# dpmerrell/PathMatFac.jl

Measured on AMD Instinct MI355X. Metric: fit_iters_per_sec, higher is better.
Workload: dtype f32; 1 GPU; fit! epoch on synthetic 200000x50000 matrix (D stored as f32), K=64, Gaussian loss, group-reg X (32 groups) + featureset-ARD Y, adam; rows sharded over 1 GPU(s); full_model=False, M=200000, N=50000, K=64, rows_per_gpu=200000, optimizer=adam, parallelism=single GPU, rccl_ranks=0, collectives_issued=0, column_chunks=1

## Files before the change

pathmatfac.jl_amd/csrc/pmf_common.h:

```cpp
#ifndef PMF_COMMON_H
#define PMF_COMMON_H
#include <hip/hip_runtime.h>

#include <cstdint>
#include <type_traits>
#include <unordered_map>

#include "../../include/pmf_hip.h"

int pmf_fail(const char *fmt, ...);
#define HIPCHK(x)                                                                                    \
  do {                                                                                               \
    hipError_t e_ = (x);                                                                             \
    if (e_ != hipSuccess) return pmf_fail("%s failed: %s (%s:%d)", #x, hipGetErrorString(e_), __FILE__, __LINE__); \
  } while (0)
#define PMFCHK(x)          \
  do {                     \
    int r_ = (x);          \
    if (r_ < 0) return r_; \
  } while (0)

typedef std::unordered_map<const void *, size_t> PmfDynLds;
int pmf_ensure_dyn_lds(PmfDynLds *cache, const void *kern, size_t lds);

// ... 29 lines not shown
  float *gY;
  float *gy_slabs;
  int64_t slab_stride;
  int64_t n_rp;
  int64_t n_tiles;
  const int64_t *wg_begin;
  int32_t tps;
  int32_t n_ct;
  const float4 *colp;
  const int32_t *bor;
  const float2 *btab;
  const float2 *btd;
  const uint8_t *pm, *row_slot, *colview;
  int32_t nbs_shift;
  int32_t n_bv;
  double *loss_partial;
  int64_t M, N;
  int32_t n_cseg;
  int32_t want_gx, want_gy;
  unsigned long long *stamps;
  int32_t dbg;
  const ViewDesc *views;
  const char *Xsb, *Ysb;
  int32_t ct0;
  float *gx_part;
  const int32_t *piece_base;
  int64_t gx_slot_stride;
  const float *sb_scale_x, *sb_scale_y;
};

__device__ __forceinline__ int pmf_rowmap(int r, int h) { return (r & 3) + 8 * (r >> 2) + 4 * h; }
__device__ __forceinline__ bool pmf_finite(float y) { return fabsf(y) <= 3.402823466e38f; }

__device__ __forceinline__ void pmf_noise(int kind, float z, float y, float w, float &l, float &g) {
  if (kind == PMF_NOISE_NORMAL) {
    const float d = z - y;
    g = w * d;
    l = 0.5f * g * d;
  } else if (kind == PMF_NOISE_BERNOULLI) {
    const float e = __expf(-fabsf(z));
    const float sp = fmaxf(z, 0.f) + __logf(1.f + e);
    const float r = __frcp_rn(1.f + e);
    const float sg = z >= 0.f ? r : e * r;
    l = w * (sp - y * z);
    g = w * (sg - y);
  } else {
// ... 249 lines not shown
```

pathmatfac.jl_amd/csrc/pmf_ctx.h:

```cpp
#ifndef PMF_CTX_H
#define PMF_CTX_H
#include <hip/hip_runtime.h>

#include <algorithm>
#include <chrono>
#include <cmath>
#include <cstdarg>
#include <cstdio>
#include <cstdlib>
#include <cstring>
#include <string>
#include <unordered_map>
#include <vector>

#include "pmf_common.h"

struct ParamBuf {
  float *p = nullptr, *g = nullptr, *acc = nullptr, *mom = nullptr;
  float *wq = nullptr, *cq = nullptr;
  float *wl1 = nullptr;
  int64_t n = 0;
  float bp1 = 0.f, bp2 = 0.f;
};

// ... 104 lines not shown
  bool has_ard = false;
  bool ard_is_fsard = false;
  int opt_kind = PMF_OPT_ADAGRAD;
  float lr = 1.f, eps = 1e-8f, b1 = 0.9f, b2 = 0.999f;
  bool state_init = false;
  double *loss_partial = nullptr;
  std::vector<uint8_t> h_kind;
  std::vector<WorkSplit> splits;
  int n_chunks_req = 0;
  float *gx_part = nullptr;
  size_t gx_part_cap = 0;
  int32_t *gx_off = nullptr, *gx_idx = nullptr;
  int64_t gx_serial = -1;
  int64_t split_serial = 0;
  Comm comm;
  int last_chunks = 1;
  hipEvent_t ev_host = nullptr;
  int64_t kind_version = 0;
  float *gy_slabs = nullptr;
  size_t gy_slabs_cap = 0;
  int precision = PMF_PREC_F32;
  char *xsb = nullptr, *ysb = nullptr;
  size_t xsb_cap = 0, ysb_cap = 0;
  float *sb8_scale = nullptr;
  uint32_t *sb8_max = nullptr;
  int64_t sb_launches = 0;
  int64_t loss_cap = 0;
  int64_t n_macro = 0;
  double *reg_partial = nullptr;
  double *d_loss = nullptr;
  double *h_loss = nullptr;
  std::vector<std::pair<hipEvent_t, hipEvent_t>> ev_pool;
  size_t ev_used = 0;
  double kernel_ms_sum = 0.0;
  int64_t kernel_launches = 0;
  NetReg *net[2] = {nullptr, nullptr};
  int reg_counts[4] = {0, 0, 0, 0};
  void *scratch = nullptr;
  size_t scratch_bytes = 0;
  PmfDynLds dyn_lds;
};

#define REG_SLOTS 1024
#define PMF_MAX_CHUNKS 16

struct FusedFamily;
// ... 61 lines not shown
```

pathmatfac.jl_amd/csrc/pmf_fused.hip.inc:

```

template <int KB, int NW, int RBW = 1>
struct FusedCfg {
  static constexpr int Kp = 32 * KB;
  static constexpr int KpS = Kp + 4;
  static constexpr int SLAB = 32 * Kp;
  static constexpr int YT = PMF_BN * KpS;
  static constexpr int XP = 32 * KpS;
  static constexpr int TT = (RBW - 1) * 1024;
  static constexpr int FIXED = NW * SLAB + NW * RBW * XP + NW * TT + 8 * PMF_BN + 4;
  static constexpr int LDS_BUDGET = 160 * 1024;
  static constexpr int NYB = (2 * YT + FIXED) * 4 + 8 * NW <= LDS_BUDGET ? 2 : 1;
  static constexpr size_t lds_bytes = (sizeof(float) * (NYB * YT + FIXED) + sizeof(double) * NW + 15) / 16 * 16;
  static constexpr size_t lds_batch_extra = PMF_BN * 16 * sizeof(float2) + PMF_PM_BYTES + NW * RBW * 16 * 32;
};

#ifndef PMF_NW4_WAVES
#define PMF_NW4_WAVES 1
#endif
template <int KB, int NW, int RBW, int BMODE, bool MIXED, int GM, bool DB, bool XW = false>
__global__ __launch_bounds__(64 * NW, (NW == 8 ? 2 : PMF_NW4_WAVES)) void pmf_fused_kernel(const FusedArgs a) {
  using Cfg = FusedCfg<KB, NW, RBW>;
  constexpr bool FULL = GM != 3;
  constexpr bool BATCH = BMODE != 0;
  constexpr bool bt_lds = BMODE == 1;
// ... 36 lines not shown
  const int dbg = FULL ? 0 : a.dbg;
  float *Sw = Sl + w * SLAB;
  float *Xw[RBW], *T[RBW];
#pragma unroll
  for (int rb = 0; rb < RBW; ++rb) {
    Xw[rb] = Xs + (w * RBW + rb) * Cfg::XP;
    T[rb] = rb == 0 ? Sw + (KB - 1) * 1024 : Tt + (w * (RBW - 1) + rb - 1) * 1024;
  }
  const int xw_j = 16 * (w & 1) + (lane & 15), xw_k = 16 * (w >> 1) + 4 * (lane >> 4);
  const int xw_e = xw_j * Kp + xw_k;
  const int xw_x = 4 * (lane >> 4) * KpS + 16 * (w >> 1) + (lane & 15);
  int xw_g[4];
  typedef const __attribute__((address_space(3))) float *lds_cptr;
  unsigned xw_xa[4];
#pragma unroll
  for (int u = 0; u < 4; ++u) {
    const int i = 4 * (lane >> 4) + u;
    xw_g[u] = i * 32 + 4 * ((xw_j >> 2) ^ (i & 7)) + (xw_j & 3);
    xw_xa[u] = (unsigned)(uintptr_t)(lds_cptr)(Xs + xw_x + u * KpS);
    if (XW) asm volatile("" : "+v"(xw_xa[u]));
  }

  constexpr bool HOIST = KB == 2 && NW == 8 && RBW == 1 && GM != 3 && (XW || GM != 0 || BMODE == 0);
  unsigned ho_y[2][YV], ho_s[2][YV], ho_c[2], ho_g[2][RV4];
  if (HOIST) {
#pragma unroll
    for (int z = 0; z < 2; ++z) {
      const int ncol = z == 0 || N % BN == 0 ? BN : (int)(N % BN);
#pragma unroll
      for (int q = 0; q < YV; ++q) {
        int e4 = tid + NT * q;
        if (e4 > BN * Kp / 4 - 1) e4 = BN * Kp / 4 - 1;
        int jl = (e4 * 4) / Kp;
        if (jl >= ncol) { jl = ncol - 1; e4 = jl * (Kp / 4); }
        ho_y[z][q] = 16u * e4;
        ho_s[z][q] = 16u * jl;
        asm volatile("" : "+v"(ho_y[z][q]), "+v"(ho_s[z][q]));
      }
      ho_c[z] = 16u * (tid < ncol ? tid : ncol - 1);
      asm volatile("" : "+v"(ho_c[z]));
#pragma unroll
      for (int q = 0; q < RV4; ++q) {
        int e = xw_e;
        if (!XW) {
          const int f = tid + NT * q, ff = f < BN * Kp / 4 ? f : 0;
          e = ((ff % (BN * 8)) / 8) * Kp + 32 * (ff / (BN * 8)) + 4 * (ff % 8);
        }
        ho_g[z][q] = 4u * (e < ncol * Kp ? e : e % Kp);
        asm volatile("" : "+v"(ho_g[z][q]));
      }
    }
  }
  auto ho_at = [](const void *base, unsigned off) { return reinterpret_cast<const char *>(base) + off; };
#ifdef PMF_STAMPS
  unsigned long long st_acc[16] = {0, 0, 0, 0, 0, 0, 0, 0, 0, 0, 0, 0, 0, 0, 0, 0};
  unsigned long long st_prev = __builtin_amdgcn_s_memtime();
  const unsigned long long st_t0 = st_prev, st_r0 = __builtin_amdgcn_s_memrealtime();
#endif
  const int wg = pmf_xcd_wg(blockIdx.x, gridDim.x);
  const int64_t w_begin = a.wg_begin[wg];
  const int64_t w_end = a.wg_begin[wg + 1];
// ... 24 lines not shown
      irow_c[rb] = row_ok[rb] ? irow : (M - 1);
    }

    constexpr int XV = (32 * Kp / 4) / 64;
    float4 xv0[RBW][XV];
#pragma unroll
    for (int rb = 0; rb < RBW; ++rb) {
#pragma unroll
      for (int q = 0; q < XV; ++q) {
        const int e4 = lane + 64 * q;
        const int il = (e4 * 4) / Kp;
        const int64_t ir = row0[rb] + il < M ? row0[rb] + il : M - 1;
        xv0[rb][q] = *reinterpret_cast<const float4 *>(a.X + ir * Kp + (e4 * 4) % Kp);
      }
    }
    f32x16 gx[RBW][KB];
#pragma unroll
    for (int rb = 0; rb < RBW; ++rb)
#pragma unroll
      for (int kb = 0; kb < KB; ++kb)
#pragma unroll
        for (int r = 0; r < 16; ++r) gx[rb][kb][r] = 0.f;

    auto stage_load_y = [&](int64_t jt, int q, float4 (&yv)[YV], float (&sgv)[YV]) {
      const float *yb = a.Y + jt * Kp;
      const float4 *cb = a.colp + jt;
      const int64_t rem = N - jt;
      if (HOIST) {
        const bool rag = rem < BN;
        yv[q] = *reinterpret_cast<const float4 *>(ho_at(yb, rag ? ho_y[1][q] : ho_y[0][q]));
        sgv[q] = *reinterpret_cast<const float *>(ho_at(cb, rag ? ho_s[1][q] : ho_s[0][q]));
        return;
      }
      const int ncol = rem > BN ? BN : (int)rem;
      int e4 = tid + NT * q;
      if (e4 > BN * Kp / 4 - 1) e4 = BN * Kp / 4 - 1;
      int jl = (e4 * 4) / Kp;
      if (jl >= ncol) { jl = ncol - 1; e4 = jl * (Kp / 4); }
      yv[q] = *reinterpret_cast<const float4 *>(yb + e4 * 4);
      sgv[q] = cb[jl].x;
    };
    auto stage_load_c = [&](int64_t jt, float4 &cv) {
      const float4 *cb = a.colp + jt;
      const int64_t rem = N - jt;
      if (HOIST) {
        cv = *reinterpret_cast<const float4 *>(ho_at(cb, rem < BN ? ho_c[1] : ho_c[0]));
        return;
      }
      const int ncol = rem > BN ? BN : (int)rem;
      cv = cb[tid < ncol ? tid : ncol - 1];
    };
    auto stage_load = [&](int64_t jt, float4 (&yv)[YV], float (&sgv)[YV], float4 &cv) {
#pragma unroll
      for (int q = 0; q < YV; ++q) stage_load_y(jt, q, yv, sgv);
      stage_load_c(jt, cv);
    };
    auto stage_store = [&](int ybuf, int cbuf, int64_t jt, const float4 (&yv)[YV], const float (&sgv)[YV], const float4 &cv) {
      float *Yn = Ys + ybuf * Cfg::YT;
      const int64_t rem = N - jt;
      const int ncol = rem > BN ? BN : (int)rem;
#pragma unroll
      for (int q = 0; q < YV; ++q) {
        const int e4 = tid + NT * q;
        if (e4 < BN * Kp / 4) {
          const int jl = (e4 * 4) / Kp, kf = (e4 * 4) % Kp;
          const float sg = jl < ncol ? sgv[q] : 0.f;
          *reinterpret_cast<float4 *>(Yn + jl * KpS + kf) = make_float4(yv[q].x * sg, yv[q].y * sg, yv[q].z * sg, yv[q].w * sg);
        }
      }
      asm volatile("" ::"v"(cv.x), "v"(cv.y), "v"(cv.z), "v"(cv.w));
      if (tid < BN) {
        const bool livec = tid < ncol;
        Csg[cbuf * BN + tid] = livec ? cv.x : 0.f;
        Cmu[cbuf * BN + tid] = livec ? cv.y : 0.f;
        Cw[cbuf * BN + tid] = livec ? cv.z : 0.f;
        Cmt[cbuf * BN + tid] = livec ? __float_as_int(cv.w) : 3;
        if (MIXED) {
          const int kd = __float_as_int(cv.w) & 3;
          const unsigned m0 = (unsigned)__ballot(!livec || kd == 0), m1 = (unsigned)__ballot(!livec || kd == 1),
                         m2 = (unsigned)__ballot(!livec || kd == 2);
          if (tid == 0) Ck[cbuf] = m0 == 0xffffffffu ? 0 : (m1 == 0xffffffffu ? 1 : (m2 == 0xffffffffu ? 2 : 3));
        }
        if (bt_lds) {
          const int vw = (__float_as_int(cv.w) >> 2) - 1;
          const int vw0 = __builtin_amdgcn_readfirstlane(vw);
          const unsigned mv = (unsigned)__ballot(!livec || vw == vw0);
          if (tid == 0) Ck[2 + cbuf] = mv == 0xffffffffu ? vw0 : -2;
        }
      }
    };
// ... 100 lines not shown
          float4 v = racc[q];
          const float sgj = Csg[(cbuf ^ 1) * BN + eo[q] / Kp];
          v.x *= sgj; v.y *= sgj; v.z *= sgj; v.w *= sgj;
          if (!slab_first) { v.x += gold[q].x; v.y += gold[q].y; v.z += gold[q].z; v.w += gold[q].w; }
          if (in[q] && eo[q] < nel) pmf_store_stream(reinterpret_cast<float4 *>(sb + eo[q]), v);
        }
      }
    };

    bool rows_in[RBW];
    int rb_u[RBW];
    uint32_t tflag[RBW];
#pragma unroll
    for (int rb = 0; rb < RBW; ++rb) {
      const int rb_raw = __builtin_amdgcn_readfirstlane((int)(row0[rb] >> 5));
      rows_in[rb] = rb_raw < a.nRB;
      rb_u[rb] = rows_in[rb] ? rb_raw : (int)a.nRB - 1;
      tflag[rb] = a.tflags[(col_begin >> 5) * a.nRB + rb_u[rb]];
#pragma unroll
      for (int q = 0; q < DCH; ++q) dcur[rb].load(a.D, (col_begin >> 5) * a.nRB + rb_u[rb], lane, q);
    }
    {
      float4 yv[YV], cv;
      float sgv[YV];
      stage_load(col_begin, yv, sgv, cv);
#pragma unroll
      for (int rb = 0; rb < RBW; ++rb)
#pragma unroll
        for (int q = 0; q < XV; ++q) {
          const int e4 = lane + 64 * q;
          const int il = (e4 * 4) / Kp, kf = (e4 * 4) % Kp;
          *reinterpret_cast<float4 *>(Xw[rb] + il * KpS + kf) = row0[rb] + il < M ? xv0[rb][q] : make_float4(0.f, 0.f, 0.f, 0.f);
        }
      stage_store(0, 0, col_begin, yv, sgv, cv);
      if (bt_lds) {
#pragma unroll
        for (int q = 0; q < NBT; ++q) {
          const int e = bt_e(q);
          bt_store(e, pmf_bt_entry(a, a.pm + rp * a.n_bv * 16, col_begin, e, pmf_bt_view(a, col_begin, e)), bt_mu(col_begin, e));
        }
        if (tid < a.n_bv * 16) Pm[tid] = a.pm[rp * a.n_bv * 16 + tid];
        if (h == 0)
#pragma unroll
          for (int rb = 0; rb < RBW; ++rb)
            for (int v = 0; v < a.n_bv; ++v) Bw0[rb * 512 + v * 32 + l31] = a.row_slot[(int64_t)v * M + irow_c[rb]];
      }
    }
    __syncthreads();

    f32x16 acc[RBW];
    forward_reduce(acc, 0, 0, false, 0);

    for (int t = 0; t < ntiles; ++t) {
      const int par = t & 1;
      const int cur = NYB == 2 ? par : 0, nxt = NYB == 2 ? (par ^ 1) : 0;
      const int64_t j0 = col_begin + (int64_t)t * BN;
      const float *Yc = Ys + cur * Cfg::YT;
      const bool have_next = (t + 1 < ntiles);
      const int cb0 = par * BN + 4 * h;
      float4 ynext[YV], cnext;
      float2 btn[NBT];
      float btm[NBT];
      int btv[NBT];
      float sgnext[YV];
      PMF_STAMP(0);
      const float xw_sg = XW ? Csg[par * BN + xw_j] : 0.f;

      float lsum = 0.f;
      const int tkind = MIXED ? __builtin_amdgcn_readfirstlane(Ck[par]) : 0;
      const int tview = bt_lds ? __builtin_amdgcn_readfirstlane(Ck[2 + par]) : -1;
      float lnorm = 0.f;
      auto epi_reg = [&](int rb, int r, float dl, float th, float wj, int kmode, bool fast) __attribute__((always_inline)) {
        if (dbg & 4) return;
        float z = acc[rb][r];
        if (BATCH) z = fmaf(z, dl, th);
        float y = dcur[rb].get(r);
        if (kmode == PMF_NOISE_NORMAL) {
          if (!fast) y = (pmf_finite(y) && row_ok[rb]) ? y : z;
          const float d = z - y, g = wj * d;
          lnorm = fmaf(g, d, lnorm);
          acc[rb][r] = BATCH ? g * dl : g;
        } else {
          const bool ok = pmf_finite(y) && row_ok[rb];
          float l, g;
          if (kmode == 3) pmf_noise(Cmt[cb0 + (r & 3) + 8 * (r >> 2)] & 3, z, y, wj, l, g);
          else pmf_noise(kmode, z, y, wj, l, g);
          lsum += ok ? l : 0.f;
          acc[rb][r] = ok ? (BATCH ? g * dl : g) : 0.f;
        }
// ... 27 lines not shown
                  tv[u] += dt.y;
                }
              }
            }
          }
          dl4 = make_float4(dv[0], dv[1], dv[2], dv[3]);
          th4 = make_float4(tv[0], tv[1], tv[2], tv[3]);
        }
      };
      const float4 *cw4 = reinterpret_cast<const float4 *>(Cw + cb0);
      auto f4get = [](const float4 &v, int u) { return u == 0 ? v.x : (u == 1 ? v.y : (u == 2 ? v.z : v.w)); };

      const int64_t jn = have_next ? j0 + BN : j0;
      constexpr int NOTH = YV + 1 + RV4 + (BATCH ? NBT : 0);
      constexpr int NVM = NOTH + (DCH + 1) * RBW;
      bool tile_fast[RBW];
#pragma unroll
      for (int rb = 0; rb < RBW; ++rb) tile_fast[rb] = rows_in[rb] && tflag[rb] != 0;
      auto vmem_op = [&](int i) {
        if (i == 0 && bt_lds) {
#pragma unroll
          for (int q = 0; q < NBT; ++q) btv[q] = pmf_bt_view(a, jn, bt_e(q));
        }
        if (i < YV) stage_load_y(jn, i, ynext, sgnext);
        else if (i == YV) stage_load_c(jn, cnext);
        else if (i < YV + 1 + RV4) { if (want_gy) slab_prefetch_one(j0, i - YV - 1); }
        else if (i < NOTH) {
          const int q = i - YV - 1 - RV4;
          if (bt_lds) { btn[q] = pmf_bt_entry(a, Pm, jn, bt_e(q), btv[q]); btm[q] = bt_mu(jn, bt_e(q)); }
        }
        else if (i < NVM) {
          const int rb = (i - NOTH) / (DCH + 1), q = (i - NOTH) % (DCH + 1);
          if (q < DCH) {
            if (FULL || !(dbg & 2)) dcur[rb].load(a.D, (jn >> 5) * a.nRB + rb_u[rb], lane, q);
          } else {
            tflag[rb] = a.tflags[(jn >> 5) * a.nRB + rb_u[rb]];
          }
        }
      };
      typedef float f32x2 __attribute__((ext_vector_type(2)));
#pragma unroll
      for (int rb = 0; rb < RBW; ++rb) {
        if (!BATCH && tile_fast[rb] && (!MIXED || tkind == 0)) {
          f32x2 ls2 = {0.f, 0.f};
          if (!(dbg & 4)) {
#pragma unroll
            for (int c4 = 0; c4 < 4; ++c4) {
// ... 92 lines not shown
            for (int kb = 0; kb < KB; ++kb)
              gy[kb] = __builtin_amdgcn_mfma_f32_32x32x2f32(av, Xw[rb][i * KpS + 32 * kb + l31], gy[kb], 0, 0, 0);
          }
        }
        if (GM == 2) {
#pragma unroll
          for (int i = 16; i < NVM; ++i) vmem_op(i);
        }
        if (!(dbg & 32)) {
#pragma unroll
          for (int kb = 0; kb < KB; ++kb)
#pragma unroll
            for (int r = 0; r < 16; ++r) Sw[kb * 1024 + pmf_rowmap(r, h) * 32 + l31] = gy[kb][r];
        } else {
          f32x16 keep = gy[0];
#pragma unroll
          for (int kb = 1; kb < KB; ++kb) keep += gy[kb];
          asm volatile("" ::"v"(keep));
        }
      }

      PMF_STAMP(4);
      if (NYB == 1) __syncthreads();
      stage_store(nxt, par ^ 1, jn, ynext, sgnext, cnext);
      PMF_STAMP(5);
      __syncthreads();
      PMF_STAMP(6);

      if (bt_lds) {
#pragma unroll
        for (int q = 0; q < NBT; ++q) bt_store(bt_e(q), btn[q], btm[q]);
      }
      slab_first = pidx == 0 || (pidx == 1 && ti0 + t < t0_first);
      if (XW) {
        typedef float f32x4 __attribute__((ext_vector_type(4)));
        constexpr int XW_RING = 8, XW_AHEAD = 6;
        const float *Gp = Sl + par * (NW * 1024);
        float xa[XW_RING], xb[XW_RING];
        auto xw_read = [&](int q) __attribute__((always_inline)) {
          const int p = q >> 3, u = (q >> 1) & 3;
#pragma unroll
          for (int hi = 0; hi < 2; ++hi) {
            xa[(q + hi) % XW_RING] = *(lds_cptr)(uintptr_t)(xw_xa[u] + 4 * (p * Cfg::XP + 16 * hi * KpS));
            xb[(q + hi) % XW_RING] = Gp[p * 1024 + xw_g[u] + 512 * hi];
          }
        };
#pragma unroll
        for (int q = 0; q < XW_AHEAD; q += 2) xw_read(q);
        f32x4 gy0 = {0.f, 0.f, 0.f, 0.f}, gy1 = {0.f, 0.f, 0.f, 0.f};
        __builtin_amdgcn_sched_barrier(0);
#pragma unroll
        for (int q = 0; q < 8 * NW; q += 2) {
          if (q + XW_AHEAD < 8 * NW) xw_read(q + XW_AHEAD);
          gy0 = __builtin_amdgcn_mfma_f32_16x16x4f32(xa[q % XW_RING], xb[q % XW_RING], gy0, 0, 0, 0);
          gy1 = __builtin_amdgcn_mfma_f32_16x16x4f32(xa[(q + 1) % XW_RING], xb[(q + 1) % XW_RING], gy1, 0, 0, 0);
          __builtin_amdgcn_sched_barrier(0);
        }
        dcur[0].touch();
        const int64_t rem = N - j0;
        const int nel = (rem > BN ? BN : (int)rem) * Kp;
        float4 v = make_float4((gy0[0] + gy1[0]) * xw_sg, (gy0[1] + gy1[1]) * xw_sg, (gy0[2] + gy1[2]) * xw_sg, (gy0[3] + gy1[3]) * xw_sg);
        if (!slab_first) { v.x += gold[0].x; v.y += gold[0].y; v.z += gold[0].z; v.w += gold[0].w; }
        if (xw_e < nel) pmf_store_stream(reinterpret_cast<float4 *>(myslab + j0 * Kp + xw_e), v);
        PMF_STAMP(4);
        forward_reduce(acc, nxt, par ^ 1, false, 0);
        PMF_STAMP(8);
        if (bt_lds) __syncthreads();
        PMF_STAMP(9);
      } else {
        if (FULL || have_next) forward_reduce(acc, nxt, par ^ 1, want_gy && !(dbg & 1), j0);
        else if (want_gy && !(dbg & 1)) { f32x16 dummy[RBW]; forward_reduce(dummy, nxt, par ^ 1, true, j0); }
        PMF_STAMP(8);
        if ((GM != 1 || bt_lds) && !(dbg & 16)) __syncthreads();
        PMF_STAMP(9);
      }
    }
    if (XW && !bt_lds) __syncthreads();

    PMF_STAMP(10);
    if (want_gx) {
      float *gp = a.gx_part + (int64_t)gx_slot * a.gx_slot_stride + (int64_t)(w * RBW) * 32 * Kp + l31;
#pragma unroll
      for (int rb = 0; rb < RBW; ++rb)
#pragma unroll
        for (int kb = 0; kb < KB; ++kb)
#pragma unroll
          for (int r = 0; r < 16; ++r) gp[(rb * 32 + pmf_rowmap(r, h)) * Kp + 32 * kb] = gx[rb][kb][r];
    }
// ... 21 lines not shown
```

pathmatfac.jl_amd/csrc/pmf_hip.hip:

```cpp
#include "pmf_ctx.h"

static thread_local std::string g_err;
int pmf_fail(const char *fmt, ...) {
  char buf[1024];
  va_list ap;
  va_start(ap, fmt);
  vsnprintf(buf, sizeof(buf), fmt, ap);
  va_end(ap);
  g_err = buf;
  return -1;
}
extern "C" const char *pmf_last_error(void) { return g_err.c_str(); }
extern "C" int pmf_version(void) { return 1; }


int ctx_bind(pmf_ctx *c) {
  if (!c) return pmf_fail("null context");
  HIPCHK(hipSetDevice(c->device));
  return 0;
}

int memset_now(void *p, int v, size_t bytes) {
  HIPCHK(hipMemset(p, v, bytes));
  HIPCHK(hipStreamSynchronize(nullptr));
// ... 16 lines not shown
  b.n = 0;
}

int pmf_ensure_dyn_lds(PmfDynLds *cache, const void *kern, size_t lds) {
  auto it = cache->find(kern);
  if (it != cache->end() && it->second >= lds) return 0;
  HIPCHK(hipFuncSetAttribute(kern, hipFuncAttributeMaxDynamicSharedMemorySize, (int)lds));
  (*cache)[kern] = lds;
  return 0;
}
int ensure_dyn_lds(pmf_ctx *c, const void *kern, size_t lds) { return pmf_ensure_dyn_lds(&c->dyn_lds, kern, lds); }

static int ensure_scratch(pmf_ctx *c, size_t bytes) {
  if (c->scratch_bytes >= bytes) return 0;
  if (c->scratch) HIPCHK(hipFree(c->scratch));
  c->scratch = nullptr;
  HIPCHK(hipMalloc(&c->scratch, bytes));
  c->scratch_bytes = bytes;
  return 0;
}

__global__ void k_fill(float *p, int64_t n, float v) {
  for (int64_t e = blockIdx.x * (int64_t)blockDim.x + threadIdx.x; e < n; e += (int64_t)gridDim.x * blockDim.x) p[e] = v;
}

__global__ void k_prepare(const float *logsigma, const float *mu, const float *colw, const int32_t *colmeta,
                          float4 *colp, int64_t N, const float *logdelta, const float *theta, float2 *btab,
                          int64_t nbt) {
  const int64_t e = blockIdx.x * (int64_t)blockDim.x + threadIdx.x;
  if (e < N) colp[e] = make_float4(expf(logsigma[e]), mu[e], colw[e], __int_as_float(colmeta[e]));
  if (e < nbt) btab[e] = make_float2(expf(logdelta[e]), theta[e]);
}

struct DenseBtabArgs {
  const int32_t *colmeta;
  const float2 *btab;
  float2 *btd;
  uint8_t *colview;
  int64_t N, Npad;
  int32_t nbs_shift;
  ViewDesc views[PMF_MAXV];
};
__global__ void k_dense_btab(const DenseBtabArgs a) {
  const int64_t e = blockIdx.x * (int64_t)blockDim.x + threadIdx.x;
  if (e >= (a.Npad << a.nbs_shift)) return;
  const int64_t j = e >> a.nbs_shift;
// ... 598 lines not shown
  HIPCHK(hipMalloc((void **)&c->d_loss, sizeof(double) * 8));
  HIPCHK(hipHostMalloc((void **)&c->h_loss, sizeof(double) * 8));
  HIPCHK(hipMalloc((void **)&c->reg_partial, sizeof(double) * 4 * REG_SLOTS));
  PMFCHK(memset_now(c->reg_partial, 0, sizeof(double) * 4 * REG_SLOTS));
  {
    const char *pe = getenv("PMF_PRECISION");
    if (pe && std::string(pe) == "bf16x3") c->precision = PMF_PREC_BF16X3;
  }
  *out = c;
  return 0;
}

extern "C" int pmf_destroy(pmf_ctx *c) {
  if (!c) return 0;
  (void)hipSetDevice(c->device);
  (void)hipStreamSynchronize(c->stream);
  for (auto &b : c->P) param_free(b);
  netreg_free(c, 0);
  netreg_free(c, 1);
  if (c->D) (void)hipFree(c->D);
  c->D = nullptr;
  dev_free(&c->tflags);
  dev_free(&c->bor); dev_free(&c->btab); dev_free(&c->btd); c->btd_cap = 0; c->btd_ok = false; dev_free(&c->colview); c->colview_cap = 0; dev_free(&c->LG); c->LG_cap = 0; dev_free(&c->lgrad_part); c->lgrad_part_cap = 0; dev_free(&c->d_views); c->views_dirty = true; dev_free(&c->d_val_view);
  dev_free(&c->colmeta); dev_free(&c->colw); dev_free(&c->colp);
  dev_free(&c->ard_alpha); dev_free(&c->ard_beta);
  comm_release(c);
  for (auto &ps : c->pslots) { dev_free(&ps.pm); dev_free(&ps.row_slot); }
  for (auto &ws : c->splits) { dev_free(&ws.wg_begin); dev_free(&ws.c_off); dev_free(&ws.c_idx); dev_free(&ws.piece_base); dev_free(&ws.d_piece_base_abs); }
  dev_free(&c->gx_part); dev_free(&c->gx_off); dev_free(&c->gx_idx);
  if (c->ev_host) (void)hipEventDestroy(c->ev_host);
  dev_free(&c->gy_slabs); dev_free(&c->xsb); dev_free(&c->ysb); dev_free(&c->sb8_scale); dev_free(&c->sb8_max); dev_free(&c->loss_partial); dev_free(&c->reg_partial); dev_free(&c->d_loss);
  if (c->h_loss) (void)hipHostFree(c->h_loss);
  if (c->scratch) (void)hipFree(c->scratch);
  for (auto &e : c->ev_pool) { (void)hipEventDestroy(e.first); (void)hipEventDestroy(e.second); }
  if (c->own_stream && c->stream) (void)hipStreamDestroy(c->stream);
  delete c;
  return 0;
}

extern "C" int pmf_set_precision(pmf_ctx *c, int mode) {
  if (!c) return pmf_fail("null context");
  if (mode != PMF_PREC_F32 && mode != PMF_PREC_BF16X3) return pmf_fail("unknown precision mode %d", mode);
  c->precision = mode;
  return 0;
}

extern "C" int pmf_get_precision(pmf_ctx *c, int *mode, int64_t *split_launches) {
// ... 26 lines not shown

static int data_shape_changed(pmf_ctx *c, int64_t M, int64_t N) {
  if (M <= 0 || N <= 0) return pmf_fail("empty data matrix (%lld x %lld)", (long long)M, (long long)N);
  if (M == c->M && N == c->N) return 0;
  c->M = M;
  c->N = N;
  for (auto &b : c->P) param_free(b);
  netreg_free(c, 0);
  netreg_free(c, 1);
  c->K = c->Kp = c->KB = 0;
  PMFCHK(param_alloc(c->P[2], N));
  PMFCHK(param_alloc(c->P[3], N));
  c->n_bv = 0;
  c->h_bor.clear();
  c->views_serial++;
  c->views.clear();
  c->views_dirty = true;
  c->val_off.clear();
  c->bvb_off.clear();
  dev_free(&c->bor); dev_free(&c->btab); dev_free(&c->btd); c->btd_cap = 0; c->btd_ok = false; dev_free(&c->colview); c->colview_cap = 0; dev_free(&c->LG); c->LG_cap = 0; dev_free(&c->lgrad_part); c->lgrad_part_cap = 0; dev_free(&c->d_views); c->views_dirty = true; dev_free(&c->d_val_view);
  PMFCHK(dev_alloc(&c->colmeta, (size_t)N));
  PMFCHK(dev_alloc(&c->colw, (size_t)N));
  PMFCHK(dev_alloc(&c->colp, (size_t)N));
  k_fill<<<nblocks(N, 256), 256, 0, c->stream>>>(c->colw, N, 1.f);
  HIPCHK(hipGetLastError());
  c->mixed = false;
  c->prepared = false;
  c->state_init = false;
  return 0;
}

static int alloc_tiled_D(pmf_ctx *c, int64_t M, int64_t N, int store) {
  const int64_t Npad = (N + PMF_DPAD - 1) / PMF_DPAD * PMF_DPAD;
  const int64_t nRB = (M + 31) / 32;
  const int64_t nfl = nRB * 32 * Npad;
  const size_t esz = store == PMF_STORE_BF16 ? 2 : 4;
  if (!(c->D && c->D_M == M && c->D_Npad == Npad && c->store == store)) {
    if (c->D) (void)hipFree(c->D);
    c->D = nullptr;
    HIPCHK(hipMalloc(&c->D, esz * (size_t)nfl));
    c->own_D = true;
    c->D_M = M;
    c->D_Npad = Npad;
    c->nRB = nRB;
  }
  c->tflags_valid = false;
// ... 860 lines not shown
      for (auto &v : abs) v += base;
      HIPCHK(hipMemcpy(ws.d_piece_base_abs, abs.data(), sizeof(int32_t) * abs.size(), hipMemcpyHostToDevice));
      base += (int32_t)ws.piece_rp.size();
    }
    std::vector<int32_t> off((size_t)g.n_rp + 1, 0), idx;
    for (int64_t rp = 0; rp < g.n_rp; ++rp) {
      idx.insert(idx.end(), lists[(size_t)rp].begin(), lists[(size_t)rp].end());
      off[(size_t)rp + 1] = (int32_t)idx.size();
    }
    if (idx.empty()) idx.push_back(0);
    PMFCHK(dev_alloc(&c->gx_off, off.size(), false));
    PMFCHK(dev_alloc(&c->gx_idx, idx.size(), false));
    HIPCHK(hipMemcpy(c->gx_off, off.data(), sizeof(int32_t) * off.size(), hipMemcpyHostToDevice));
    HIPCHK(hipMemcpy(c->gx_idx, idx.data(), sizeof(int32_t) * idx.size(), hipMemcpyHostToDevice));
    const size_t need = (size_t)base * (size_t)f.BM() * (size_t)c->Kp;
    if (need > c->gx_part_cap) {
      dev_free(&c->gx_part);
      PMFCHK(dev_alloc(&c->gx_part, need, false));
      c->gx_part_cap = need;
    }
    c->gx_serial = serial_sum;
  }
  PMFCHK(ensure_tile_flags(c));
  if (f.img != IMG_NONE) {
    size_t xblk = 0, yblk = 0;
    for (const FusedFamily &o : fused_families)
      if (o.img_kb == f.img_kb) { xblk = std::max<size_t>(xblk, o.xblk); yblk = std::max<size_t>(yblk, o.yblk); }
    const size_t xb = ((size_t)c->nRB + PMF_XSB_PAD) * xblk, yb = (size_t)g.n_ct_all * yblk;
    if (xb > c->xsb_cap) { dev_free(&c->xsb); c->xsb_cap = 0; PMFCHK(dev_alloc(&c->xsb, xb, true)); c->xsb_cap = xb; }
    if (yb > c->ysb_cap) { dev_free(&c->ysb); c->ysb_cap = 0; PMFCHK(dev_alloc(&c->ysb, yb, false)); c->ysb_cap = yb; }
    if (f.img == IMG_SB8 && !c->sb8_scale) {
      PMFCHK(dev_alloc(&c->sb8_scale, (size_t)(1 + PMF_MAX_CHUNKS), false));
      PMFCHK(dev_alloc(&c->sb8_max, (size_t)(1 + PMF_MAX_CHUNKS)));
    }
  }
  return 0;
}

static int sb8_split(pmf_ctx *c, const FusedFamily &f, const float *src, const float4 *colp, int64_t n, int64_t nblk, int slot,
                     int transposed, char *out) {
  Sb8ScaleArgs sa = {src, colp, n, c->Kp, c->sb8_max + slot, c->sb8_scale + slot};
  PMFCHK(pmf_launch_sb8_scale(c->stream, sa));
  Sb8SplitArgs sp = {src, colp, c->sb8_scale + slot, n, nblk, transposed, out};
  return pmf_launch_sb8_split(c->stream, sp, f.KB);
}
static int sb_split_x(pmf_ctx *c, const FusedFamily &f) {
  if (f.img == IMG_SB8) {
    return sb8_split(c, f, c->P[0].p, nullptr, c->M, (c->nRB + f.nblk - 1) / f.nblk * f.nblk, 0, 1, c->xsb);
  }
  if (f.img == IMG_SB4) {
    Sb4SplitArgs s4 = {c->P[0].p, nullptr, c->M, c->nRB, c->Kp, 1, c->xsb};
    return pmf_launch_sb4_split(c->stream, s4);
  }
  SbSplitArgs sx = {c->P[0].p, nullptr, c->M, c->nRB, c->xsb};
  return f.KB == 1 ? pmf_launch_sb_split_1(c->stream, sx) : pmf_launch_sb_split_2(c->stream, sx);
}
static int sb_split_y(pmf_ctx *c, const FusedFamily &f, int64_t ct0, int64_t nct, int chunk) {
  const int64_t c0 = ct0 * 32;
  const float *src = c->P[1].p + c0 * c->Kp;
  char *out = c->ysb + (size_t)ct0 * (size_t)f.yblk;
  if (f.img == IMG_SB8) return sb8_split(c, f, src, c->colp + c0, std::min<int64_t>(c->N - c0, nct * 32), nct, 1 + chunk, 0, out);
  if (f.img == IMG_SB4) {
    Sb4SplitArgs s4 = {src, c->colp + c0, c->N - c0, nct, c->Kp, 0, out};
    return pmf_launch_sb4_split(c->stream, s4);
  }
  SbSplitArgs sy = {src, c->colp + c0, c->N - c0, nct, out};
  return f.KB == 1 ? pmf_launch_sb_split_1(c->stream, sy) : pmf_launch_sb_split_2(c->stream, sy);
}

int launch_fused_chunk(pmf_ctx *c, const FusedGeom &g, int s, bool want_gx, bool want_gy) {
  const FusedFamily &f = *g.fam;
  WorkSplit &ws = c->splits[(size_t)s];
  const int grid = ws.grid;
  int grid_dummy; int64_t tiles_per_seg, n_cseg;
  chunk_segments(c, g, s, grid_dummy, tiles_per_seg, n_cseg);
  const int64_t n_ct = g.nct[s], n_rp = g.n_rp;
  const int64_t slab_stride = (int64_t)c->Kp * c->N;
  int64_t loss_off = 0;
  for (int q = 0; q < s; ++q) loss_off += c->splits[(size_t)q].grid;
  FusedArgs a;
  memset(&a, 0, sizeof(a));
  a.tflags = c->tflags;
  a.wg_begin = ws.wg_begin;
  a.D = c->D; a.X = c->P[0].p; a.Y = c->P[1].p; a.gX = c->P[0].g; a.gY = c->P[1].g;
  a.colp = c->colp; a.bor = c->bor; a.btab = c->btab; a.loss_partial = c->loss_partial + loss_off;
  a.btd = g.bmode == 1 ? c->btd : nullptr; a.n_bv = c->n_bv;
  if (g.bmode == 1) {
    a.pm = g.ps->pm; a.row_slot = g.ps->row_slot; a.colview = c->colview;
    a.nbs_shift = 0;
    while ((1 << a.nbs_shift) < c->nbs) ++a.nbs_shift;
// ... 4 lines not shown
  a.want_gx = want_gx; a.want_gy = want_gy;
  a.ct0 = (int32_t)g.ct0[s];
  a.gx_part = c->gx_part; a.piece_base = ws.d_piece_base_abs; a.gx_slot_stride = (int64_t)f.BM() * c->Kp;
  {
    const char *dbg = getenv("PMF_DEBUG_FLAGS");
    a.dbg = dbg ? atoi(dbg) : 0;
  }
#ifdef PMF_STAMPS
  {
    static unsigned long long *d_stamps = nullptr;
    if (!d_stamps) HIPCHK(hipMalloc((void **)&d_stamps, sizeof(unsigned long long) * 16 * 8 * 1024));
    HIPCHK(hipMemsetAsync(d_stamps, 0, sizeof(unsigned long long) * 16 * 8 * 1024, c->stream));
    a.stamps = d_stamps;
    g_stamps = d_stamps;
  }
#endif
  a.views = c->d_views;
  const bool batch = c->n_bv > 0;
  if (f.img != IMG_NONE) {
    if (s == 0) PMFCHK(sb_split_x(c, f));
    PMFCHK(sb_split_y(c, f, g.ct0[s], n_ct, s));
    a.Xsb = c->xsb; a.Ysb = c->ysb;
    if (f.img == IMG_SB8) { a.sb_scale_x = c->sb8_scale; a.sb_scale_y = c->sb8_scale + 1 + s; }
  }
  if (c->ev_used == c->ev_pool.size()) {
    if (c->ev_pool.size() >= 4096) {
      HIPCHK(hipStreamSynchronize(c->stream));
      harvest_events(c);
    } else {
      hipEvent_t e0, e1;
      HIPCHK(hipEventCreate(&e0));
      HIPCHK(hipEventCreate(&e1));
      c->ev_pool.emplace_back(e0, e1);
    }
  }
  auto &ev = c->ev_pool[c->ev_used++];
  HIPCHK(hipEventRecord(ev.first, c->stream));
  c->last_kernel = f.kernel;
  const int rc = f.launch[c->store == PMF_STORE_BF16](&c->dyn_lds, c->stream, a, grid, batch, c->mixed);
  if (f.kernel != 0) c->sb_launches += 1;
  PMFCHK(rc);
  HIPCHK(hipEventRecord(ev.second, c->stream));
  if (want_gy && !(a.dbg & 8)) {
    k_gy_reduce<<<dim3((unsigned)n_ct, (unsigned)(32 * c->Kp / 256)), 64, 0, c->stream>>>(c->gy_slabs, slab_stride, ws.c_off, ws.c_idx,
                                                                                      c->Kp, c->N, c->P[1].g, (int)g.ct0[s],
                                                                                      f.img == IMG_SB8 ? c->colp : nullptr);
// ... 411 lines not shown
```

Baseline: 31.19 iters/s.

## Prescale Y by column sigma in a separate kernel and interleave X-weight and forward MFMA

A small pre-pass kernel writes Y multiplied by each column's sigma into a padded buffer. The fused kernel then loads plain float4 tiles with no per-column scale loads, ragged-edge index math or multiplies, and the two-set hoisted offsets shrink to one. The gY (XW) MFMA loop is also reworked: X reads are issued before the barrier, the mu accumulator init and the first Y/X forward operands are prefetched inside the loop, and the slab store is interleaved with the forward 32x32 MFMA chain instead of calling forward_reduce. The trade-off is an extra launch plus a write and read of an N×Kp buffer each chunk, and higher register pressure.

Result: no change. 31.35 iters/s (median of 6 runs) (+0.5%).

```diff
diff --git a/pathmatfac.jl_amd/csrc/pmf_common.h b/pathmatfac.jl_amd/csrc/pmf_common.h
--- a/pathmatfac.jl_amd/csrc/pmf_common.h
+++ b/pathmatfac.jl_amd/csrc/pmf_common.h
@@ -75,6 +75,7 @@
   int32_t dbg;
   const ViewDesc *views;
   const char *Xsb, *Ysb;
+  const float *Ysc;
   int32_t ct0;
   float *gx_part;
   const int32_t *piece_base;
diff --git a/pathmatfac.jl_amd/csrc/pmf_ctx.h b/pathmatfac.jl_amd/csrc/pmf_ctx.h
--- a/pathmatfac.jl_amd/csrc/pmf_ctx.h
+++ b/pathmatfac.jl_amd/csrc/pmf_ctx.h
@@ -150,6 +150,8 @@
   int precision = PMF_PREC_F32;
   char *xsb = nullptr, *ysb = nullptr;
   size_t xsb_cap = 0, ysb_cap = 0;
+  float *ysc = nullptr;
+  size_t ysc_cap = 0;
   float *sb8_scale = nullptr;
   uint32_t *sb8_max = nullptr;
   int64_t sb_launches = 0;
diff --git a/pathmatfac.jl_amd/csrc/pmf_fused.hip.inc b/pathmatfac.jl_amd/csrc/pmf_fused.hip.inc
--- a/pathmatfac.jl_amd/csrc/pmf_fused.hip.inc
+++ b/pathmatfac.jl_amd/csrc/pmf_fused.hip.inc
@@ -82,21 +82,18 @@
   }
 
   constexpr bool HOIST = KB == 2 && NW == 8 && RBW == 1 && GM != 3 && (XW || GM != 0 || BMODE == 0);
-  unsigned ho_y[2][YV], ho_s[2][YV], ho_c[2], ho_g[2][RV4];
+  unsigned ho_y[YV], ho_c[2], ho_g[2][RV4];
   if (HOIST) {
+#pragma unroll
+    for (int q = 0; q < YV; ++q) {
+      int e4 = tid + NT * q;
+      if (e4 > BN * Kp / 4 - 1) e4 = BN * Kp / 4 - 1;
+      ho_y[q] = 16u * e4;
+      asm volatile("" : "+v"(ho_y[q]));
+    }
 #pragma unroll
     for (int z = 0; z < 2; ++z) {
       const int ncol = z == 0 || N % BN == 0 ? BN : (int)(N % BN);
-#pragma unroll
-      for (int q = 0; q < YV; ++q) {
-        int e4 = tid + NT * q;
-        if (e4 > BN * Kp / 4 - 1) e4 = BN * Kp / 4 - 1;
-        int jl = (e4 * 4) / Kp;
-        if (jl >= ncol) { jl = ncol - 1; e4 = jl * (Kp / 4); }
-        ho_y[z][q] = 16u * e4;
-        ho_s[z][q] = 16u * jl;
-        asm volatile("" : "+v"(ho_y[z][q]), "+v"(ho_s[z][q]));
-      }
       ho_c[z] = 16u * (tid < ncol ? tid : ncol - 1);
       asm volatile("" : "+v"(ho_c[z]));
 #pragma unroll
@@ -167,23 +164,15 @@
 #pragma unroll
         for (int r = 0; r < 16; ++r) gx[rb][kb][r] = 0.f;
 
-    auto stage_load_y = [&](int64_t jt, int q, float4 (&yv)[YV], float (&sgv)[YV]) {
-      const float *yb = a.Y + jt * Kp;
-      const float4 *cb = a.colp + jt;
-      const int64_t rem = N - jt;
+    auto stage_load_y = [&](int64_t jt, int q, float4 (&yv)[YV]) {
+      const float *yb = a.Ysc + jt * Kp;
       if (HOIST) {
-        const bool rag = rem < BN;
-        yv[q] = *reinterpret_cast<const float4 *>(ho_at(yb, rag ? ho_y[1][q] : ho_y[0][q]));
-        sgv[q] = *reinterpret_cast<const float *>(ho_at(cb, rag ? ho_s[1][q] : ho_s[0][q]));
+        yv[q] = *reinterpret_cast<const float4 *>(ho_at(yb, ho_y[q]));
         return;
       }
-      const int ncol = rem > BN ? BN : (int)rem;
       int e4 = tid + NT * q;
       if (e4 > BN * Kp / 4 - 1) e4 = BN * Kp / 4 - 1;
-      int jl = (e4 * 4) / Kp;
-      if (jl >= ncol) { jl = ncol - 1; e4 = jl * (Kp / 4); }
       yv[q] = *reinterpret_cast<const float4 *>(yb + e4 * 4);
-      sgv[q] = cb[jl].x;
     };
     auto stage_load_c = [&](int64_t jt, float4 &cv) {
       const float4 *cb = a.colp + jt;
@@ -195,12 +184,12 @@
       const int ncol = rem > BN ? BN : (int)rem;
       cv = cb[tid < ncol ? tid : ncol - 1];
     };
-    auto stage_load = [&](int64_t jt, float4 (&yv)[YV], float (&sgv)[YV], float4 &cv) {
-#pragma unroll
-      for (int q = 0; q < YV; ++q) stage_load_y(jt, q, yv, sgv);
+    auto stage_load = [&](int64_t jt, float4 (&yv)[YV], float4 &cv) {
+#pragma unroll
+      for (int q = 0; q < YV; ++q) stage_load_y(jt, q, yv);
       stage_load_c(jt, cv);
     };
-    auto stage_store = [&](int ybuf, int cbuf, int64_t jt, const float4 (&yv)[YV], const float (&sgv)[YV], const float4 &cv) {
+    auto stage_store = [&](int ybuf, int cbuf, int64_t jt, const float4 (&yv)[YV], const float4 &cv) {
       float *Yn = Ys + ybuf * Cfg::YT;
       const int64_t rem = N - jt;
       const int ncol = rem > BN ? BN : (int)rem;
@@ -209,8 +198,7 @@
         const int e4 = tid + NT * q;
         if (e4 < BN * Kp / 4) {
           const int jl = (e4 * 4) / Kp, kf = (e4 * 4) % Kp;
-          const float sg = jl < ncol ? sgv[q] : 0.f;
-          *reinterpret_cast<float4 *>(Yn + jl * KpS + kf) = make_float4(yv[q].x * sg, yv[q].y * sg, yv[q].z * sg, yv[q].w * sg);
+          *reinterpret_cast<float4 *>(Yn + jl * KpS + kf) = yv[q];
         }
       }
       asm volatile("" ::"v"(cv.x), "v"(cv.y), "v"(cv.z), "v"(cv.w));
@@ -357,8 +345,7 @@
     }
     {
       float4 yv[YV], cv;
-      float sgv[YV];
-      stage_load(col_begin, yv, sgv, cv);
+      stage_load(col_begin, yv, cv);
 #pragma unroll
       for (int rb = 0; rb < RBW; ++rb)
 #pragma unroll
@@ -367,7 +354,7 @@
           const int il = (e4 * 4) / Kp, kf = (e4 * 4) % Kp;
           *reinterpret_cast<float4 *>(Xw[rb] + il * KpS + kf) = row0[rb] + il < M ? xv0[rb][q] : make_float4(0.f, 0.f, 0.f, 0.f);
         }
-      stage_store(0, 0, col_begin, yv, sgv, cv);
+      stage_store(0, 0, col_begin, yv, cv);
       if (bt_lds) {
 #pragma unroll
         for (int q = 0; q < NBT; ++q) {
@@ -397,9 +384,22 @@
       float2 btn[NBT];
       float btm[NBT];
       int btv[NBT];
-      float sgnext[YV];
       PMF_STAMP(0);
       const float xw_sg = XW ? Csg[par * BN + xw_j] : 0.f;
+      typedef float f32x4 __attribute__((ext_vector_type(4)));
+      constexpr int XW_RING = 8, XW_AHEAD = 6;
+      const float *Gp = Sl + par * (NW * 1024);
+      float xa[XW_RING], xb[XW_RING];
+      auto xw_read_x = [&](int q) __attribute__((always_inline)) {
+        const int p = q >> 3, u = (q >> 1) & 3;
+#pragma unroll
+        for (int hi = 0; hi < 2; ++hi) xa[(q + hi) % XW_RING] = *(lds_cptr)(uintptr_t)(xw_xa[u] + 4 * (p * Cfg::XP + 16 * hi * KpS));
+      };
+      auto xw_read_g = [&](int q) __attribute__((always_inline)) {
+        const int p = q >> 3, u = (q >> 1) & 3;
+#pragma unroll
+        for (int hi = 0; hi < 2; ++hi) xb[(q + hi) % XW_RING] = Gp[p * 1024 + xw_g[u] + 512 * hi];
+      };
 
       float lsum = 0.f;
       const int tkind = MIXED ? __builtin_amdgcn_readfirstlane(Ck[par]) : 0;
@@ -473,7 +473,7 @@
 #pragma unroll
           for (int q = 0; q < NBT; ++q) btv[q] = pmf_bt_view(a, jn, bt_e(q));
         }
-        if (i < YV) stage_load_y(jn, i, ynext, sgnext);
+        if (i < YV) stage_load_y(jn, i, ynext);
         else if (i == YV) stage_load_c(jn, cnext);
         else if (i < YV + 1 + RV4) { if (want_gy) slab_prefetch_one(j0, i - YV - 1); }
         else if (i < NOTH) {
@@ -612,8 +612,12 @@
 
       PMF_STAMP(4);
       if (NYB == 1) __syncthreads();
-      stage_store(nxt, par ^ 1, jn, ynext, sgnext, cnext);
+      stage_store(nxt, par ^ 1, jn, ynext, cnext);
       PMF_STAMP(5);
+      if (XW) {
+#pragma unroll
+        for (int q = 0; q < XW_AHEAD; q += 2) xw_read_x(q);
+      }
       __syncthreads();
       PMF_STAMP(6);
 
@@ -623,37 +627,52 @@
       }
       slab_first = pidx == 0 || (pidx == 1 && ti0 + t < t0_first);
       if (XW) {
-        typedef float f32x4 __attribute__((ext_vector_type(4)));
-        constexpr int XW_RING = 8, XW_AHEAD = 6;
-        const float *Gp = Sl + par * (NW * 1024);
-        float xa[XW_RING], xb[XW_RING];
-        auto xw_read = [&](int q) __attribute__((always_inline)) {
-          const int p = q >> 3, u = (q >> 1) & 3;
-#pragma unroll
-          for (int hi = 0; hi < 2; ++hi) {
-            xa[(q + hi) % XW_RING] = *(lds_cptr)(uintptr_t)(xw_xa[u] + 4 * (p * Cfg::XP + 16 * hi * KpS));
-            xb[(q + hi) % XW_RING] = Gp[p * 1024 + xw_g[u] + 512 * hi];
+#pragma unroll
+        for (int q = 0; q < XW_AHEAD; q += 2) xw_read_g(q);
+        f32x4 gy0 = {0.f, 0.f, 0.f, 0.f}, gy1 = {0.f, 0.f, 0.f, 0.f};
+        const float4 *fyr = reinterpret_cast<const float4 *>(Ys + nxt * Cfg::YT + l31 * KpS + h * (Kp / 2));
+        const float4 *fxr = reinterpret_cast<const float4 *>(Xw[0] + l31 * KpS + h * (Kp / 2));
+        const float4 *fmu = reinterpret_cast<const float4 *>(Cmu + (par ^ 1) * BN + 4 * h);
+        float4 fyv, fxv;
+        __builtin_amdgcn_sched_barrier(0);
+#pragma unroll
+        for (int q = 0; q < 8 * NW; q += 2) {
+          if (q + XW_AHEAD < 8 * NW) { xw_read_x(q + XW_AHEAD); xw_read_g(q + XW_AHEAD); }
+          if (q == 8 * NW - 6) {
+#pragma unroll
+            for (int c4 = 0; c4 < 4; ++c4) {
+              const float4 m4 = BATCH ? make_float4(0.f, 0.f, 0.f, 0.f) : fmu[2 * c4];
+              acc[0][4 * c4] = m4.x; acc[0][4 * c4 + 1] = m4.y; acc[0][4 * c4 + 2] = m4.z; acc[0][4 * c4 + 3] = m4.w;
+            }
           }
-        };
-#pragma unroll
-        for (int q = 0; q < XW_AHEAD; q += 2) xw_read(q);
-        f32x4 gy0 = {0.f, 0.f, 0.f, 0.f}, gy1 = {0.f, 0.f, 0.f, 0.f};
-        __builtin_amdgcn_sched_barrier(0);
-#pragma unroll
-        for (int q = 0; q < 8 * NW; q += 2) {
-          if (q + XW_AHEAD < 8 * NW) xw_read(q + XW_AHEAD);
+          if (q == 8 * NW - 4) fyv = fyr[0];
+          if (q == 8 * NW - 2) fxv = fxr[0];
           gy0 = __builtin_amdgcn_mfma_f32_16x16x4f32(xa[q % XW_RING], xb[q % XW_RING], gy0, 0, 0, 0);
           gy1 = __builtin_amdgcn_mfma_f32_16x16x4f32(xa[(q + 1) % XW_RING], xb[(q + 1) % XW_RING], gy1, 0, 0, 0);
           __builtin_amdgcn_sched_barrier(0);
         }
-        dcur[0].touch();
-        const int64_t rem = N - j0;
-        const int nel = (rem > BN ? BN : (int)rem) * Kp;
-        float4 v = make_float4((gy0[0] + gy1[0]) * xw_sg, (gy0[1] + gy1[1]) * xw_sg, (gy0[2] + gy1[2]) * xw_sg, (gy0[3] + gy1[3]) * xw_sg);
-        if (!slab_first) { v.x += gold[0].x; v.y += gold[0].y; v.z += gold[0].z; v.w += gold[0].w; }
-        if (xw_e < nel) pmf_store_stream(reinterpret_cast<float4 *>(myslab + j0 * Kp + xw_e), v);
         PMF_STAMP(4);
-        forward_reduce(acc, nxt, par ^ 1, false, 0);
+        constexpr int NIT = KS / 4;
+#pragma unroll
+        for (int q = 0; q < NIT; ++q) {
+          float4 yn = fyv, xn = fxv;
+          if (q + 1 < NIT) { yn = fyr[q + 1]; xn = fxr[q + 1]; }
+          acc[0] = __builtin_amdgcn_mfma_f32_32x32x2f32(fyv.x, fxv.x, acc[0], 0, 0, 0);
+          acc[0] = __builtin_amdgcn_mfma_f32_32x32x2f32(fyv.y, fxv.y, acc[0], 0, 0, 0);
+          acc[0] = __builtin_amdgcn_mfma_f32_32x32x2f32(fyv.z, fxv.z, acc[0], 0, 0, 0);
+          acc[0] = __builtin_amdgcn_mfma_f32_32x32x2f32(fyv.w, fxv.w, acc[0], 0, 0, 0);
+          if (q == 0) {
+            dcur[0].touch();
+            asm volatile("" ::"v"(tflag[0]));
+            const int64_t rem = N - j0;
+            const int nel = (rem > BN ? BN : (int)rem) * Kp;
+            float4 v = make_float4((gy0[0] + gy1[0]) * xw_sg, (gy0[1] + gy1[1]) * xw_sg, (gy0[2] + gy1[2]) * xw_sg, (gy0[3] + gy1[3]) * xw_sg);
+            if (!slab_first) { v.x += gold[0].x; v.y += gold[0].y; v.z += gold[0].z; v.w += gold[0].w; }
+            if (xw_e < nel) pmf_store_stream(reinterpret_cast<float4 *>(myslab + j0 * Kp + xw_e), v);
+          }
+          fyv = yn; fxv = xn;
+          __builtin_amdgcn_sched_barrier(0);
+        }
         PMF_STAMP(8);
         if (bt_lds) __syncthreads();
         PMF_STAMP(9);
diff --git a/pathmatfac.jl_amd/csrc/pmf_hip.hip b/pathmatfac.jl_amd/csrc/pmf_hip.hip
--- a/pathmatfac.jl_amd/csrc/pmf_hip.hip
+++ b/pathmatfac.jl_amd/csrc/pmf_hip.hip
@@ -62,6 +62,19 @@
 
 __global__ void k_fill(float *p, int64_t n, float v) {
   for (int64_t e = blockIdx.x * (int64_t)blockDim.x + threadIdx.x; e < n; e += (int64_t)gridDim.x * blockDim.x) p[e] = v;
+}
+
+__global__ void k_y_scale(const float4 *Y, const float4 *colp, int64_t ncols, int64_t n4, int kp4, float4 *out) {
+  const int64_t e = blockIdx.x * (int64_t)blockDim.x + threadIdx.x;
+  if (e >= n4) return;
+  const int64_t j = e / kp4;
+  float4 v = make_float4(0.f, 0.f, 0.f, 0.f);
+  if (j < ncols) {
+    const float sg = colp[j].x;
+    const float4 y = Y[e];
+    v = make_float4(y.x * sg, y.y * sg, y.z * sg, y.w * sg);
+  }
+  out[e] = v;
 }
 
 __global__ void k_prepare(const float *logsigma, const float *mu, const float *colw, const int32_t *colmeta,
@@ -706,7 +719,7 @@
   c->D = nullptr;
   dev_free(&c->tflags);
   dev_free(&c->bor); dev_free(&c->btab); dev_free(&c->btd); c->btd_cap = 0; c->btd_ok = false; dev_free(&c->colview); c->colview_cap = 0; dev_free(&c->LG); c->LG_cap = 0; dev_free(&c->lgrad_part); c->lgrad_part_cap = 0; dev_free(&c->d_views); c->views_dirty = true; dev_free(&c->d_val_view);
-  dev_free(&c->colmeta); dev_free(&c->colw); dev_free(&c->colp);
+  dev_free(&c->colmeta); dev_free(&c->colw); dev_free(&c->colp); dev_free(&c->ysc); c->ysc_cap = 0;
   dev_free(&c->ard_alpha); dev_free(&c->ard_beta);
   comm_release(c);
   for (auto &ps : c->pslots) { dev_free(&ps.pm); dev_free(&ps.row_slot); }
@@ -779,6 +792,7 @@
   PMFCHK(dev_alloc(&c->colmeta, (size_t)N));
   PMFCHK(dev_alloc(&c->colw, (size_t)N));
   PMFCHK(dev_alloc(&c->colp, (size_t)N));
+  dev_free(&c->ysc); c->ysc_cap = 0;
   k_fill<<<nblocks(N, 256), 256, 0, c->stream>>>(c->colw, N, 1.f);
   HIPCHK(hipGetLastError());
   c->mixed = false;
@@ -1685,6 +1699,10 @@
     c->gx_serial = serial_sum;
   }
   PMFCHK(ensure_tile_flags(c));
+  if (f.img == IMG_NONE) {
+    const size_t yn = (size_t)g.n_ct_all * PMF_BN * (size_t)c->Kp;
+    if (yn > c->ysc_cap) { dev_free(&c->ysc); c->ysc_cap = 0; PMFCHK(dev_alloc(&c->ysc, yn, false)); c->ysc_cap = yn; }
+  }
   if (f.img != IMG_NONE) {
     size_t xblk = 0, yblk = 0;
     for (const FusedFamily &o : fused_families)
@@ -1729,6 +1747,14 @@
   }
   SbSplitArgs sy = {src, c->colp + c0, c->N - c0, nct, out};
   return f.KB == 1 ? pmf_launch_sb_split_1(c->stream, sy) : pmf_launch_sb_split_2(c->stream, sy);
+}
+
+static int y_scale(pmf_ctx *c, int64_t ct0, int64_t nct) {
+  const int64_t c0 = ct0 * PMF_BN, n4 = nct * PMF_BN * (c->Kp / 4);
+  k_y_scale<<<nblocks(n4, 256), 256, 0, c->stream>>>(reinterpret_cast<const float4 *>(c->P[1].p + c0 * c->Kp), c->colp + c0, c->N - c0, n4,
+                                                    c->Kp / 4, reinterpret_cast<float4 *>(c->ysc + c0 * c->Kp));
+  HIPCHK(hipGetLastError());
+  return 0;
 }
 
 int launch_fused_chunk(pmf_ctx *c, const FusedGeom &g, int s, bool want_gx, bool want_gy) {
@@ -1779,6 +1805,9 @@
     PMFCHK(sb_split_y(c, f, g.ct0[s], n_ct, s));
     a.Xsb = c->xsb; a.Ysb = c->ysb;
     if (f.img == IMG_SB8) { a.sb_scale_x = c->sb8_scale; a.sb_scale_y = c->sb8_scale + 1 + s; }
+  } else {
+    PMFCHK(y_scale(c, g.ct0[s], n_ct));
+    a.Ysc = c->ysc;
   }
   if (c->ev_used == c->ev_pool.size()) {
     if (c->ev_pool.size() >= 4096) {
```
